# taiyaki-go/motioncheck_ccm_slam

Measured on AMD Instinct MI355X. Metric: ORB extract+match Mfeatures/s and GBA iter/s (2k KF, 200k pts) @1/2/4/8 GPU, higher is better.
Workload: dtype u8; 1 GPU; configs[1]: 256 synthetic 752x480 frames per GPU, 8-level pyramid, 1000 features, FAST+quadtree+rBRIEF, then 1000x1000 brute-force Hamming on the 255 consecutive pairs; frames_per_gpu=256

## Files before the change

motioncheck_ccm_slam_amd/csrc/orb_fast_cells.hip:

```cpp
#include <hip/hip_runtime.h>
#include "orb_types.h"
#include "orb_device.h"

#ifndef FC_NZ
#define FC_NZ 1024
#endif
#ifndef FC_KEPT
#define FC_KEPT 480
#endif
#define FC_CELLS 32
#ifndef FC_TPB
#define FC_TPB 256
#endif
static_assert(FC_TPB == FC_ITEM_STRIDE, "the band record carries the item steps of FC_WAVES waves (fc_enum, orb_device.h)");
#define FC_WAVE_CAP 320
__host__ __device__ inline size_t fc_lds_bytes(int pitch, int bh)
{
    return 2 * (size_t)pitch * bh + (size_t)FC_WAVE_CAP * (FC_TPB / 64) * 2 + 32 + FC_NZ * 2 + FC_KEPT * 4 + FC_CELLS * 16 + 64 * 8 + 256 + 64;
}

__device__ __forceinline__ unsigned fc_u(fc_us2 x) { return __builtin_bit_cast(unsigned, x); }
__device__ __forceinline__ int fc_mbcnt(unsigned long long m, int base)
{
    return (int)__builtin_amdgcn_mbcnt_hi((unsigned)(m >> 32), __builtin_amdgcn_mbcnt_lo((unsigned)m, (unsigned)base));
}
#ifdef FC_STAMPS
#define FC_STAMP_SLOTS 16
#define FC_STAMP_WGS (1 << 17)
__device__ unsigned long long fc_stamps[FC_STAMP_WGS * FC_STAMP_SLOTS];
#define FC_STAMP(k) do { if (threadIdx.x == 0 || threadIdx.x == FC_TPB - 1) { const unsigned wg__ = blockIdx.y * gridDim.x + blockIdx.x; if (wg__ < FC_STAMP_WGS) fc_stamps[wg__ * FC_STAMP_SLOTS + (threadIdx.x ? 8 : 0) + (k)] = __builtin_amdgcn_s_memtime(); } } while (0)
extern "C" int ccm_debug_fc_stamps(unsigned long long* out, int n_wgs)
{
    return hipMemcpyFromSymbol(out, HIP_SYMBOL(fc_stamps), (size_t)n_wgs * FC_STAMP_SLOTS * 8, 0, hipMemcpyDeviceToHost) == hipSuccess ? 0 : -1;
}
#else
#define FC_STAMP(k) do { } while (0)
#endif
typedef const __attribute__((address_space(1))) uint8_t fc_gbyte;
typedef const __attribute__((address_space(1))) unsigned fc_gu32;
typedef const __attribute__((address_space(3))) uint8_t fc_lbyte;
typedef unsigned fc_u32x4 __attribute__((ext_vector_type(4)));
typedef fc_u32x4 fc_u32x4_a4 __attribute__((aligned(4)));
struct FcLate {
    int ini_th, min_th, ncells, slots_per_frame;
    const OrbCell* cells; unsigned* slots; int* cell_count;
    int* clear_status;
};
__global__ __launch_bounds__(FC_TPB) __attribute__((amdgpu_waves_per_eu(8, 8))) void k_fast_cells(const OrbBand* __restrict__ bands, int xcd_on, unsigned grid_x, unsigned grid_y, int frame0,
                                                    const uint8_t* __restrict__ img0, long long plane0, int pitch0, const FcLate g)
{
    extern __shared__ __attribute__((aligned(16))) uint8_t fc_smem[];
    int wx, wy;
    xcd_work_item(xcd_on, grid_x, grid_y, wx, wy);
    FC_STAMP(0);
    const OrbBand B = bands[wx];
#ifdef FC_STAMPS
    asm volatile("s_waitcnt lgkmcnt(0)" ::: "memory");
#endif
    FC_STAMP(6);
    int bclo[4], bcwd[4], bsfirst[4], bscap[4];
#pragma unroll
    for (int i = 0; i < 4; i++) {
        bclo[i] = B.clo[i]; bcwd[i] = B.cwd[i]; bsfirst[i] = B.slot_first[i]; bscap[i] = B.slot_cap[i];
        asm volatile("" : "+s"(bclo[i]), "+s"(bcwd[i]), "+s"(bsfirst[i]), "+s"(bscap[i]));
    }
    int bxa = B.xa, by0 = B.y0, bncells = B.ncells, bcfirst = B.cell_first;
    asm volatile("" : "+s"(bxa), "+s"(by0), "+s"(bncells), "+s"(bcfirst));
    unsigned pw_inv = B.pw_inv, pq_inv = B.pq_inv;
    asm volatile("" : "+s"(pw_inv), "+s"(pq_inv));
    const int f = wy + frame0, tid = threadIdx.x, lane = lane_id(), wv = tid >> 6;
    const bool lvl0 = B.level == 0;
    const uint8_t* const Limg = lvl0 ? img0 : B.img;
    const long long Lplane = lvl0 ? plane0 : B.plane;
    const int Lpitch = lvl0 ? pitch0 : B.lpitch, Lw = B.w, Lh = B.h;
    const int P = B.pitch, bh = B.bh, PW = P >> 2;
    uint8_t* T = fc_smem;
    uint8_t* S = fc_smem + (size_t)P * bh;
    constexpr int NW = FC_TPB / 64;
    const int WCAP = FC_WAVE_CAP;
    unsigned short* surv = reinterpret_cast<unsigned short*>(S + (size_t)P * bh);
    int* nsurv = reinterpret_cast<int*>(surv + NW * WCAP);
    unsigned short* nz = reinterpret_cast<unsigned short*>(nsurv + 8);
    unsigned* kept = reinterpret_cast<unsigned*>(nz + FC_NZ);
    int* cell_hi = reinterpret_cast<int*>(kept + FC_KEPT);
    int* cell_n = cell_hi + FC_CELLS;
    int* cell_k = cell_n + FC_CELLS;
    uint2* colmask = reinterpret_cast<uint2*>(cell_k + FC_CELLS + FC_CELLS);
    uint8_t* colcell = reinterpret_cast<uint8_t*>(colmask + 64);
    int* l_clo = reinterpret_cast<int*>(colcell + 256); int* l_cwd = l_clo + 4; int* l_sfirst = l_cwd + 4; int* l_scap = l_sfirst + 4;
    const uint8_t* img = Limg + (long long)f * Lplane;
    const bool dword_ok = ((reinterpret_cast<uintptr_t>(img) | (uintptr_t)Lpitch) & 3) == 0 && Lpitch >= ((Lw + 3) & ~3);
#ifdef FC_STAMPS
    asm volatile("s_waitcnt lgkmcnt(0)" ::: "memory");
#endif
    FC_STAMP(5);
    fc_gbyte* const gimg = (fc_gbyte*)img;
    const OrbBand* const brec = bands + wx;
    auto under_trip = [&]() {
        if (g.clear_status && (blockIdx.x | blockIdx.y | threadIdx.x) == 0) *g.clear_status = 0;
        const int k = FC_TPB - 1 - tid;
        if (k < FC_CELLS) {
            cell_hi[k] = 0; cell_n[k] = 0; cell_k[k] = 0;
            if (k < 2) nsurv[1 + k] = 0;
            if (k < ORB_BAND_CELLS) { l_clo[k] = brec->clo[k]; l_cwd[k] = brec->cwd[k]; l_sfirst[k] = brec->slot_first[k]; l_scap[k] = brec->slot_cap[k]; }
        }
    };
    if (dword_ok && (P & 15) == 0) {
        const int wmax = ((Lw - 1) & ~3);
        const int PQ = P >> 4, nq = bh * PQ;
        auto chunk = [&](int i) {
            const int ly = (int)(((unsigned)i * pq_inv) >> 20), lq = i - ly * PQ;
            const int gy = min(B.y0 + ly, Lh - 1), gx = B.xa + 16 * lq;
            fc_gbyte* rowp = gimg + (long long)gy * Lpitch;
            fc_u32x4 v;
            if (gx + 12 <= wmax) v = *reinterpret_cast<const __attribute__((address_space(1))) fc_u32x4_a4*>(rowp + gx);
            else {
                v.x = *reinterpret_cast<fc_gu32*>(rowp + min(gx, wmax));
                v.y = *reinterpret_cast<fc_gu32*>(rowp + min(gx + 4, wmax));
                v.z = *reinterpret_cast<fc_gu32*>(rowp + min(gx + 8, wmax));
                v.w = *reinterpret_cast<fc_gu32*>(rowp + min(gx + 12, wmax));
            }
            return v;
        };
        fc_u32x4 v0 = { 0u, 0u, 0u, 0u };
        if (tid < nq) v0 = chunk(tid);
        asm volatile("" ::: "memory");
        under_trip();
        if (tid < nq) {
            reinterpret_cast<fc_u32x4*>(T)[tid] = v0;
            reinterpret_cast<uint4*>(S)[tid] = make_uint4(0u, 0u, 0u, 0u);
        }
        for (int i = tid + FC_TPB; i < nq; i += FC_TPB) {
            const fc_u32x4 v = chunk(i);
            reinterpret_cast<fc_u32x4*>(T)[i] = v;
            reinterpret_cast<uint4*>(S)[i] = make_uint4(0u, 0u, 0u, 0u);
        }
    } else if (dword_ok) {
        const int wmax = ((Lw - 1) & ~3);
        for (int i = tid; i < bh * PW; i += FC_TPB) {
            const int ly = (int)(((unsigned)i * pw_inv) >> 20), lx = i - ly * PW;
            const int gy = min(B.y0 + ly, Lh - 1), gx = min(B.xa + 4 * lx, wmax);
            reinterpret_cast<unsigned*>(T)[i] = *reinterpret_cast<fc_gu32*>(gimg + (long long)gy * Lpitch + gx);
            reinterpret_cast<unsigned*>(S)[i] = 0u;
        }
        under_trip();
    } else {
        for (int i = tid; i < bh * P; i += FC_TPB) {
            const int ly = i / P, lx = i - ly * P;
            const int gy = min(B.y0 + ly, Lh - 1), gx = min(B.xa + lx, Lw - 1);
            T[i] = gimg[(long long)gy * Lpitch + gx];
            S[i] = 0;
        }
        under_trip();
    }
#ifdef FC_STAMPS
    asm volatile("s_waitcnt vmcnt(0)" ::: "memory");
#endif
    FC_STAMP(7);
    const int c_lo = B.c_lo, c_hi = B.c_hi;
    const int t_lo = min(g.ini_th, g.min_th);
    const int dw_lo = B.dw_lo;
    if (tid < PW) {
        unsigned mk[4];
        for (int i = 0; i < 4; i++) mk[i] = (4 * tid + i >= c_lo && 4 * tid + i < c_hi) ? 0xFFFFu : 0u;
        colmask[tid] = make_uint2(mk[0] | (mk[2] << 16), mk[1] | (mk[3] << 16));
    }
    __syncthreads();
    FC_STAMP(1);
    if (tid < P) {
        int ci = 255;
#pragma unroll
        for (int i = 0; i < ORB_BAND_CELLS; i++) if (i < bncells && tid >= bclo[i] && tid < bclo[i] + bcwd[i]) ci = i;
        colcell[tid] = (uint8_t)ci;
    }
    const int wvs = __builtin_amdgcn_readfirstlane(wv);
    unsigned short* wsurv = surv + wvs * WCAP;
    const unsigned t_lds = (unsigned)(uintptr_t)(fc_lbyte*)T;
    const int thr = max(t_lo, 1);
    int wcnt = 0;
    auto score_top = [&]() {
        wcnt = __builtin_amdgcn_readfirstlane(wcnt);
        const int n = min(wcnt, 64);
        wcnt -= n;
        const bool on = lane < n;
        const unsigned long long on_mask = n >= 64 ? ~0ull : (1ull << n) - 1ull;
        const unsigned popped = wsurv[wcnt + lane];
        const unsigned ent = on ? popped : (unsigned)(3 * P + 3);
        const int pos = (int)(ent & 0x7FFFu);
        int rb[7];
#pragma unroll
        for (int k = 0; k < 7; k++) rb[k] = pos + (int)(t_lds + (unsigned)((k - 3) * P - 3));
#define FC_PX(dx, dy) (*(fc_lbyte*)(uintptr_t)(unsigned)(rb[(dy) + 3] + ((dx) + 3)))
        const int v = FC_PX(0, 0);
        int r[16];
        r[0] = FC_PX(0, 3);    r[1] = FC_PX(1, 3);    r[2] = FC_PX(2, 2);    r[3] = FC_PX(3, 1);
        r[4] = FC_PX(3, 0);    r[5] = FC_PX(3, -1);   r[6] = FC_PX(2, -2);   r[7] = FC_PX(1, -3);
        r[8] = FC_PX(0, -3);   r[9] = FC_PX(-1, -3);  r[10] = FC_PX(-2, -2); r[11] = FC_PX(-3, -1);
        r[12] = FC_PX(-3, 0);  r[13] = FC_PX(-3, 1);  r[14] = FC_PX(-2, 2);  r[15] = FC_PX(-1, 3);
#undef FC_PX
        auto store = [&](bool st, int arc) {
            if (st) {
                S[pos] = (uint8_t)(arc - 1);
                const int q = atomicAdd(nsurv + 1, 1);
                if (q < FC_NZ) nz[q] = (unsigned short)pos;
            }
        };
        if (t_lo < 0) {
            const int arc = fast_score16(v, r) + 1;
            store(on && arc > thr, arc);
            return;
        }
        bool again;
        const int arc = fast_arc16_split(v, r, t_lo, (ent >> 15) != 0u, &again);
        store(on && arc > thr, arc);
        const unsigned long long mb = __ballot(again) & on_mask;
        if (mb != 0ull) {
            if (on && again) wsurv[fc_mbcnt(mb, wcnt)] = (unsigned short)(ent | 0x8000u);
            wcnt += __popcll(mb);
            __builtin_amdgcn_fence(__ATOMIC_RELEASE, "wavefront");
        }
    };
    {
        const int n_dw = B.items.n_dw, d_step = B.items.d_step, r_step = B.items.r_step;
        const int runs = fc_item_runs(bh, n_dw), dw_end = dw_lo + n_dw;
        FcItem item = fc_item_start(dw_lo, n_dw, B.items.nd_inv, wv, lane);
        for (int run = wvs; run < runs; run += FC_WAVES) {
            wcnt = __builtin_amdgcn_readfirstlane(wcnt);
            const int pos0 = fc_item_pos0(item, P);
            unsigned kk0 = 0, kk1 = 0;
            if (fc_item_valid(item, bh)) {
                const unsigned* crow = reinterpret_cast<const unsigned*>(T + pos0);
                const unsigned c0 = crow[-1], c1 = crow[0], c2 = crow[1];
                const unsigned nn = crow[3 * PW], ss = crow[-3 * PW];
                const fc_us2 tt = fc_pk((unsigned)t_lo * 0x00010001u);
                unsigned kk[2];
#pragma unroll
                for (int h = 0; h < 2; h++) {
                    const unsigned sel = h ? 0x0c030c01u : 0x0c020c00u;
                    const fc_us2 v = fc_pk(__builtin_amdgcn_perm(0u, c1, sel));
                    const fc_us2 n = fc_pk(__builtin_amdgcn_perm(0u, nn, sel)), sq = fc_pk(__builtin_amdgcn_perm(0u, ss, sel));
                    const fc_us2 w = fc_pk(__builtin_amdgcn_perm(c1, c0, h ? 0x0c040c02u : 0x0c030c01u));
                    const fc_us2 e = fc_pk(__builtin_amdgcn_perm(c2, c1, h ? 0x0c060c04u : 0x0c050c03u));
                    const fc_us2 bm = __builtin_elementwise_min(__builtin_elementwise_max(n, sq), __builtin_elementwise_max(e, w));
                    const fc_us2 dm = __builtin_elementwise_max(__builtin_elementwise_min(n, sq), __builtin_elementwise_min(e, w));
                    kk[h] = fc_u(__builtin_elementwise_sub_sat(bm, (fc_us2)(v + tt))) | fc_u(__builtin_elementwise_sub_sat(__builtin_elementwise_sub_sat(v, tt), dm));
                }
                const uint2 cm = colmask[item.dw];
                kk0 = kk[0] & cm.x; kk1 = kk[1] & cm.y;
            }
            fc_item_step(item, dw_end, n_dw, d_step, r_step);
            const bool k0 = (kk0 & 0xFFFFu) != 0u, k1 = (kk1 & 0xFFFFu) != 0u;
            const bool k2 = (kk0 >> 16) != 0u, k3 = (kk1 >> 16) != 0u;
            const unsigned long long m0 = __ballot(k0), m1 = __ballot(k1), m2 = __ballot(k2), m3 = __ballot(k3);
            if ((m0 | m1 | m2 | m3) != 0ull) {
                const int b1 = wcnt + __popcll(m0), b2 = b1 + __popcll(m1), b3 = b2 + __popcll(m2);
                if (k0) (wsurv + wcnt)[fc_mbcnt(m0, 0)] = (unsigned short)pos0;
                if (k1) (wsurv + b1)[fc_mbcnt(m1, 0)] = (unsigned short)(pos0 + 1);
                if (k2) (wsurv + b2)[fc_mbcnt(m2, 0)] = (unsigned short)(pos0 + 2);
                if (k3) (wsurv + b3)[fc_mbcnt(m3, 0)] = (unsigned short)(pos0 + 3);
                wcnt = b3 + __popcll(m3);
                __builtin_amdgcn_fence(__ATOMIC_RELEASE, "wavefront");
            }
            const int leave = run + FC_WAVES < runs ? 63 : 0;
            while (wcnt > leave) score_top();
        }
    }
    __syncthreads();
    FC_STAMP(2);
    const int nnz = nsurv[1];
    const int rh = bh - 6;
    bool listed = g.min_th <= g.ini_th && nnz <= FC_NZ && bncells <= ORB_BAND_CELLS;
    if (listed) {
        const int cap_c = ((FC_KEPT / max(bncells, 1)) - 1) | 1;
        const unsigned p_inv = 0xFFFFFFFFu / (unsigned)P + 1u;
        for (int e = tid; e < nnz; e += FC_TPB) {
            const int pos = nz[e];
            const int row = (int)__umulhi((unsigned)pos, p_inv), col = pos - row * P;
            const uint8_t* p = S + pos;
            const int ci = colcell[col];
            const int sc = p[0];
            const int nl = p[-1], nr = p[1], nul = p[-P - 1], nu = p[-P], nur = p[-P + 1], ndl = p[P - 1], nd = p[P], ndr = p[P + 1];
            __builtin_amdgcn_sched_barrier(0);
            if (ci == 255) continue;
            const int xx = col - l_clo[ci], yy = row - 3, rw = l_cwd[ci];
            const bool l = xx > 0, r = xx + 1 < rw, u = yy > 0, d = yy + 1 < rh;
#define NB(c, v) ((c) ? (v) : 0)
            const bool keep = (sc > NB(l, nl)) & (sc > NB(r, nr)) &
                              (sc > NB(u && l, nul)) & (sc > NB(u, nu)) & (sc > NB(u && r, nur)) &
                              (sc > NB(d && l, ndl)) & (sc > NB(d, nd)) & (sc > NB(d && r, ndr));
#undef NB
            if (keep) {
                const int q = atomicAdd(cell_k + ci, 1);
                if (q < cap_c) kept[ci * cap_c + q] = ((unsigned)yy << 14) | ((unsigned)xx << 8) | (unsigned)sc;
                if (sc >= g.ini_th) atomicAdd(cell_hi + ci, 1);
            }
        }
        __syncthreads();
        FC_STAMP(3);
        const int4 ck = *reinterpret_cast<const int4*>(cell_k);
        const int e1 = ck.x, e2 = e1 + ck.y, e3 = e2 + ck.z, nk = e3 + ck.w;
        listed = max(max(ck.x, ck.y), max(ck.z, ck.w)) <= cap_c;
        if (listed) {
            if (tid >= FC_TPB - FC_CELLS && FC_TPB - 1 - tid < bncells) {
                const int ci = FC_TPB - 1 - tid;
                const int hi = cell_hi[ci];
                g.cell_count[(long long)f * g.ncells + bcfirst + ci] = hi > 0 ? hi : cell_k[ci];
            }
            for (int e = tid; e < nk; e += FC_TPB) {
                const int ci = (e >= e1 ? 1 : 0) + (e >= e2 ? 1 : 0) + (e >= e3 ? 1 : 0);
                const int k0 = e - (ci == 0 ? 0 : ci == 1 ? e1 : ci == 2 ? e2 : e3);
                const unsigned* bucket = kept + ci * cap_c;
                const int nb = ci == 0 ? ck.x : ci == 1 ? ck.y : ci == 2 ? ck.z : ck.w;
                const unsigned me = bucket[k0];
                const unsigned th = (unsigned)(cell_hi[ci] > 0 ? g.ini_th : g.min_th);
                if ((me & 255u) < th) continue;
                int rank = 0;
                for (int k = 0; k < nb; k++) {
                    const unsigned o = bucket[k];
                    rank += ((o & 255u) >= th && (o >> 8) < (me >> 8)) ? 1 : 0;
                }
                if (rank < l_scap[ci])
                    g.slots[(long long)f * g.slots_per_frame + l_sfirst[ci] + rank] =
                        ((me & 255u) << 24) | ((unsigned)(by0 + 3 - ORB_BORDER + (int)((me >> 14) & 63u)) << 12) |
                        (unsigned)(bxa + l_clo[ci] - ORB_BORDER + (int)((me >> 8) & 63u));
            }
            FC_STAMP(4);
            return;
        }
    }
    for (int ci = wv; ci < B.ncells; ci += FC_TPB / 64) {
        const OrbCell c = g.cells[B.cell_first + ci];
        const int rw = c.cw - 6, rh = c.ch - 6;
        int* count_out = g.cell_count + (long long)f * g.ncells + B.cell_first + ci;
        if (rw <= 0 || rh <= 0) { if (lane == 0) *count_out = 0; continue; }
        const uint8_t* S0 = S + 3 * P + (c.x0 + 3 - B.xa);
        unsigned* out = g.slots + (long long)f * g.slots_per_frame + c.slot_first;
        const int relx = c.x0 + 3 - ORB_BORDER, rely = c.y0 + 3 - ORB_BORDER;
        const int rpi = rw <= 32 ? 2 : 1;
        const int xx = rpi == 2 ? (lane & 31) : lane, yoff = rpi == 2 ? (lane >> 5) : 0;
        int n = 0;
        for (int attempt = 0; attempt < 2 && n == 0; attempt++) {
            const int th = attempt == 0 ? g.ini_th : g.min_th;
            for (int y0 = 0; y0 < rh; y0 += rpi) {
                const int yy = y0 + yoff;
                const bool in = yy < rh && xx < rw;
                const uint8_t* p = S0 + min(yy, rh - 1) * P + min(xx, rw - 1);
                const int s = in ? p[0] : 0;
                if (__ballot(s >= th && s > 0) == 0ull) continue;
                bool keep = false;
                if (s >= th && s > 0) {
                    const bool l = xx > 0, r = xx + 1 < rw, u = yy > 0, d = yy + 1 < rh;
#define NB(c, o) ((c) && (int)p[o] >= th ? (int)p[o] : 0)
                    keep = s > NB(l, -1) && s > NB(r, 1) &&
                           s > NB(u && l, -P - 1) && s > NB(u, -P) && s > NB(u && r, -P + 1) &&
                           s > NB(d && l, P - 1) && s > NB(d, P) && s > NB(d && r, P + 1);
#undef NB
                }
                const unsigned long long m = __ballot(keep);
                if (keep) {
                    const int pos = n + __popcll(m & lanemask_lt());
                    if (pos < c.slot_cap)
                        out[pos] = ((unsigned)s << 24) | ((unsigned)(rely + yy) << 12) | (unsigned)(relx + xx);
                }
                n += __popcll(m);
            }
        }
        if (lane == 0) *count_out = n;
    }
}

void orb_launch_fast_cells(hipStream_t s, const OrbGeom& g_dev, const OrbCell* cells, const OrbBand* bands, int nbands, int nframes,
                           size_t lds_bytes, unsigned* slots, int* cell_count, int* clear_status)
{
    static const int xcd_on = getenv("CCM_ORB_XCD") ? atoi(getenv("CCM_ORB_XCD")) : 0;
    const FcLate late = { g_dev.ini_th, g_dev.min_th, g_dev.ncells, g_dev.slots_per_frame, cells, slots, cell_count, clear_status };
    hipLaunchKernelGGL(k_fast_cells, dim3(nbands, nframes), dim3(FC_TPB), lds_bytes, s, bands, xcd_on, (unsigned)nbands, (unsigned)nframes, g_dev.frame0,
                       g_dev.lv[0].img, g_dev.lv[0].plane, g_dev.lv[0].pitch, late);
}
size_t orb_fast_cells_lds(int pitch, int bh) { return fc_lds_bytes(pitch, bh); }
```

motioncheck_ccm_slam_amd/csrc/orb_host.cpp:

```cpp
#include "ccm_internal.h"
#include "orb_types.h"
#include "orb_device.h"
#include <cmath>
#include <cfloat>
#include <algorithm>

namespace {

inline int cv_round(float v) { return (int)lrintf(v); }
inline int cv_round(double v) { return (int)lrint(v); }

struct OrbTables {
    float scale[ORB_MAX_LEVELS], inv_scale[ORB_MAX_LEVELS], sigma2[ORB_MAX_LEVELS], inv_sigma2[ORB_MAX_LEVELS];
    int nfeat[ORB_MAX_LEVELS];
    int umax[16];
};

int make_tables(const ccm_orb_params* p, OrbTables* t)
{
    if (!p || p->nlevels < 1 || p->nlevels > ORB_MAX_LEVELS || p->nfeatures < 0 || !(p->scale_factor > 1.0f)) return CCM_E_ARG;
    const int n = p->nlevels;
    t->scale[0] = 1.0f; t->sigma2[0] = 1.0f;
    for (int i = 1; i < n; i++) {
        t->scale[i] = t->scale[i - 1] * p->scale_factor;
// ... 129 lines not shown
        L.splane = (long long)L.spitch * L.h;
        S.smap_off[l] = smap_bytes; smap_bytes += align_up((size_t)L.splane * nframes, 256);
        if (l > 0) {
            L.pitch = (int)align_up(L.w, 64);
            L.plane = (long long)L.pitch * L.h;
            S.pyr_off[l] = pyr_bytes; pyr_bytes += align_up((size_t)L.plane * nframes, 256);
            std::vector<int> xo, yo; std::vector<short> xa, ya;
            linear_tables(G.lv[l - 1].w, L.w, xo, xa);
            linear_tables(G.lv[l - 1].h, L.h, yo, ya);
            toff[l].xofs = tab_i.size(); tab_i.insert(tab_i.end(), xo.begin(), xo.end());
            toff[l].yofs = tab_i.size(); tab_i.insert(tab_i.end(), yo.begin(), yo.end());
            toff[l].xab = tab_s.size(); tab_s.insert(tab_s.end(), xa.begin(), xa.end());
            toff[l].yab = tab_s.size(); tab_s.insert(tab_s.end(), ya.begin(), ya.end());
        }
        const int minBX = ORB_BORDER, minBY = ORB_BORDER, maxBX = L.w - ORB_EDGE + 3, maxBY = L.h - ORB_EDGE + 3;
        const float width = (float)(maxBX - minBX), height = (float)(maxBY - minBY);
        const int nCols = (int)(width / 30.f), nRows = (int)(height / 30.f);
        L.bw = maxBX - minBX; L.bh = maxBY - minBY;
        L.cell_first = (int)S.cells.size();
        int key_cap = 0;
        if (nCols >= 1 && nRows >= 1) {
            const int wCell = (int)std::ceil(width / nCols), hCell = (int)std::ceil(height / nRows);
            for (int i = 0; i < nRows; i++) {
                const float iniY = (float)(minBY + i * hCell);
                float maxY = iniY + hCell + 6;
                if (iniY >= maxBY - 3) continue;
                if (maxY > maxBY) maxY = (float)maxBY;
                for (int j = 0; j < nCols; j++) {
                    const float iniX = (float)(minBX + j * wCell);
                    float maxX = iniX + wCell + 6;
                    if (iniX >= maxBX - 6) continue;
                    if (maxX > maxBX) maxX = (float)maxBX;
                    OrbCell cell{};
                    cell.level = (short)l; cell.x0 = (short)iniX; cell.y0 = (short)iniY;
                    cell.cw = (short)((int)maxX - (int)iniX); cell.ch = (short)((int)maxY - (int)iniY);
                    if (cell.cw > 65 || cell.ch > 65)
                        return ccm_fail(c, CCM_E_ARG, "FAST cell %dx%d exceeds the kernel tile", cell.cw, cell.ch);
                    const int rw = std::max(cell.cw - 6, 0), rh = std::max(cell.ch - 6, 0);
                    cell.slot_cap = ((rw + 1) / 2) * ((rh + 1) / 2);
                    cell.slot_first = slot_acc;
                    slot_acc += cell.slot_cap; key_cap += cell.slot_cap;
                    S.cells.push_back(cell);
                }
            }
        }
        L.ncells = (int)S.cells.size() - L.cell_first;
        L.roots = (int)std::round((float)(maxBX - minBX) / (maxBY - minBY));
        if (L.roots < 1 || L.roots > ORB_MAX_ROOTS)
            return ccm_fail(c, CCM_E_ARG, "level %d aspect ratio gives %d quadtree roots (1..%d supported)", l, L.roots, ORB_MAX_ROOTS);
        L.hx = (float)(maxBX - minBX) / L.roots;
        L.key_first = key_acc; L.key_cap = std::max(key_cap, 1); key_acc += L.key_cap;
        L.out_cap = std::max(L.quota + 4, 4 * L.roots);
        L.out_first = out_acc; out_acc += L.out_cap;
        L.tiles_x = (L.w + 63) / 64; L.tiles_y = (L.h + 63) / 64;
        L.tile_first = tile_acc; tile_acc += L.tiles_x * L.tiles_y;
    }
    S.bands.clear(); S.band_lds = 0;
    static const bool want_fused = !(getenv("CCM_ORB_FUSED") && atoi(getenv("CCM_ORB_FUSED")) == 0);
    S.fused = want_fused;
    constexpr int pcap = 144;
    for (size_t a = 0; a < S.cells.size();) {
        size_t b = a;
        const OrbCell& c0 = S.cells[a];
        const int xa = (c0.x0 - 4) & ~3;
        int pitch = 0;
        while (b < S.cells.size() && S.cells[b].level == c0.level && S.cells[b].y0 == c0.y0) {
            const int p2 = (int)align_up((size_t)(S.cells[b].x0 + S.cells[b].cw + 4 - xa), 16);
            if (b > a && (p2 > pcap || b - a >= ORB_BAND_CELLS)) break;
            pitch = p2; b++;
        }
        OrbBand band{};
        band.cell_first = (int)a; band.ncells = (int)(b - a); band.level = c0.level; band.xa = (short)xa; band.y0 = (short)c0.y0;
        band.pitch = (short)pitch; band.bh = (short)c0.ch;
        {
            const OrbCell& cl = S.cells[b - 1];
            const int PW = pitch / 4, PQ = std::max(pitch / 16, 1);
            band.c_lo = (short)(c0.x0 + 3 - xa); band.c_hi = (short)(cl.x0 + cl.cw - 3 - xa);
            band.dw_lo = (short)std::max(1, band.c_lo >> 2); band.dw_hi = (short)std::min(PW - 2, (band.c_hi - 1) >> 2);
            band.pw_inv = (1u << 20) / (unsigned)PW + 1u; band.pq_inv = (1u << 20) / (unsigned)PQ + 1u;
            band.items = fc_enum(band.dw_lo, band.dw_hi);
            band.w = G.lv[c0.level].w; band.h = G.lv[c0.level].h;
            for (size_t k = a; k < b; k++) {
                const OrbCell& ck = S.cells[k];
                band.clo[k - a] = (short)(ck.x0 + 3 - xa); band.cwd[k - a] = (short)(ck.cw - 6);
                band.slot_first[k - a] = ck.slot_first; band.slot_cap[k - a] = ck.slot_cap;
            }
        }
        for (size_t k = a; k < b; k++) if (S.cells[k].ch != c0.ch) S.fused = false;
        S.bands.push_back(band);
        a = b;
    }
    for (const OrbBand& b : S.bands) S.band_lds = std::max(S.band_lds, orb_fast_cells_lds(b.pitch, b.bh));
    for (const OrbBand& b : S.bands) if (b.pitch > 256) S.fused = false;
    if (S.band_lds > 60 * 1024) S.fused = false;
    for (const OrbBand& b : S.bands) if ((int)b.pitch * b.bh >= (1 << 15)) S.fused = false;
    G.ncells = (int)S.cells.size(); G.ntiles = tile_acc;
    G.slots_per_frame = std::max(slot_acc, 1); G.keys_per_frame = key_acc; G.out_per_frame = out_acc;
    int list_cap = 0;
    for (int l = 0; l < p->nlevels; l++) list_cap = std::max(list_cap, G.lv[l].out_cap);
    G.list_cap = (int)align_up(list_cap + 4, 16);
    if (orb_octree_lds_bytes(G.list_cap) > 150 * 1024)
        return ccm_fail(c, CCM_E_ARG, "nfeatures too large for the quadtree kernel's LDS (list cap %d)", G.list_cap);
    if (max_per_image < 1) return ccm_fail(c, CCM_E_ARG, "max_per_image must be positive");

    CCM_RESERVE(c, S.pyr, std::max<size_t>(pyr_bytes, 256));
    CCM_RESERVE(c, S.smap, smap_bytes);
    CCM_RESERVE(c, S.slots, (size_t)G.slots_per_frame * nframes * 4);
    CCM_RESERVE(c, S.cell_count, (size_t)std::max(G.ncells, 1) * nframes * 4);
    CCM_RESERVE(c, S.keysA, (size_t)G.keys_per_frame * nframes * 4);
    CCM_RESERVE(c, S.keysB, (size_t)G.keys_per_frame * nframes * 4);
    CCM_RESERVE(c, S.sel, (size_t)G.out_per_frame * nframes * 4);
    CCM_RESERVE(c, S.sel_count, (size_t)p->nlevels * nframes * 4);
    CCM_RESERVE(c, S.status, 256);
    CCM_RESERVE(c, S.kps, (size_t)nframes * max_per_image * sizeof(ccm_keypoint));
    CCM_RESERVE(c, S.desc, (size_t)nframes * max_per_image * 32);
    CCM_RESERVE(c, S.counts, (size_t)nframes * 4);
    const size_t tab_bytes = align_up(tab_i.size() * 4, 16) + tab_s.size() * 2;
    CCM_RESERVE(c, S.tables_dev, std::max<size_t>(tab_bytes, 16));
    CCM_RESERVE(c, S.cells_dev, std::max<size_t>(S.cells.size(), 1) * sizeof(OrbCell));
    CCM_RESERVE(c, S.bands_dev, std::max<size_t>(S.bands.size(), 1) * sizeof(OrbBand));
    CCM_RESERVE(c, S.geom_dev, sizeof(OrbGeom));
    char* tb = S.tables_dev.as<char>();
    const size_t s_base = align_up(tab_i.size() * 4, 16);
    for (int l = 0; l < p->nlevels; l++) {
        OrbLevel& L = G.lv[l];
        L.smap = S.smap.as<uint8_t>() + S.smap_off[l];
        if (l > 0) {
            L.img = S.pyr.as<uint8_t>() + S.pyr_off[l];
            L.xofs = reinterpret_cast<const int*>(tb) + toff[l].xofs;
            L.yofs = reinterpret_cast<const int*>(tb) + toff[l].yofs;
            L.xab = reinterpret_cast<const short*>(tb + s_base) + toff[l].xab;
            L.yab = reinterpret_cast<const short*>(tb + s_base) + toff[l].yab;
        }
    }
    if (!tab_i.empty()) CCM_HIP(c, hipMemcpyAsync(tb, tab_i.data(), tab_i.size() * 4, hipMemcpyHostToDevice, c->stream));
    if (!tab_s.empty()) CCM_HIP(c, hipMemcpyAsync(tb + s_base, tab_s.data(), tab_s.size() * 2, hipMemcpyHostToDevice, c->stream));
    if (!S.cells.empty())
        CCM_HIP(c, hipMemcpyAsync(S.cells_dev.p, S.cells.data(), S.cells.size() * sizeof(OrbCell), hipMemcpyHostToDevice, c->stream));
    for (OrbBand& b : S.bands) {
        const OrbLevel& L = G.lv[b.level];
        b.img = b.level > 0 ? L.img : nullptr; b.plane = L.plane; b.lpitch = L.pitch;
    }
    if (!S.bands.empty())
        CCM_HIP(c, hipMemcpyAsync(S.bands_dev.p, S.bands.data(), S.bands.size() * sizeof(OrbBand), hipMemcpyHostToDevice, c->stream));
    CCM_HIP(c, hipStreamSynchronize(c->stream));
    if (!S.pattern_up) { CCM_HIP(c, orb_upload_pattern()); S.pattern_up = true; }
    S.par = *p; S.w = w; S.h = h; S.nframes = nframes; S.max_per_image = max_per_image;
    S.valid = true;
    S.last_img = nullptr;
    return CCM_OK;
}

static int orb_run(ccm_ctx* c, const uint8_t* img_dev, int stride, size_t image_stride, int frame0 = 0, int nrun = -1,
                   hipStream_t st = nullptr, hipEvent_t first_done = nullptr)
{
    OrbState& S = *c->orb;
    OrbGeom& G = S.geom;
    G.lv[0].img = img_dev; G.lv[0].pitch = stride; G.lv[0].plane = (long long)image_stride;
    G.frame0 = frame0;
    if (nrun < 0) nrun = S.nframes - frame0;
    if (!st) st = c->stream;
    const OrbGeom& gd = G;
    const OrbCell* cd = S.cells_dev.as<OrbCell>();
    int* clear = frame0 == 0 ? S.status.as<int>() : nullptr;
    for (int l = 1; l < G.nlevels; l++) {
        ProfScope ps(c, CCM_PROF_RESIZE);
        orb_launch_resize(st, gd, l, G.lv[l].w, G.lv[l].h, nrun, clear);
        clear = nullptr;
        if (l == 1 && first_done) CCM_HIP(c, hipEventRecord(first_done, st));
    }
    if (S.fused && !S.bands.empty()) {
        ProfScope ps(c, CCM_PROF_FAST_SCORE);
        orb_launch_fast_cells(st, gd, cd, S.bands_dev.as<OrbBand>(), (int)S.bands.size(), nrun, S.band_lds, S.slots.as<unsigned>(), S.cell_count.as<int>(), clear);
        if (G.nlevels == 1 && first_done) CCM_HIP(c, hipEventRecord(first_done, st));
    } else {
        if (clear) CCM_HIP(c, hipMemsetAsync(clear, 0, 4, st));
        { ProfScope ps(c, CCM_PROF_FAST_SCORE); orb_launch_score(st, gd, G.ntiles, nrun); }
        if (G.ncells > 0) { ProfScope ps(c, CCM_PROF_CELL_NMS); orb_launch_nms(st, gd, cd, G.ncells, nrun, S.slots.as<unsigned>(), S.cell_count.as<int>()); }
    }
    { ProfScope ps(c, CCM_PROF_OCTREE);
    orb_launch_octree(st, gd, cd, G.nlevels, nrun, G.list_cap, S.slots.as<unsigned>(), S.cell_count.as<int>(),
                      S.keysA.as<unsigned>(), S.keysB.as<unsigned>(), S.sel.as<unsigned>(), S.sel_count.as<int>(),
                      S.status.as<int>()); }
    { ProfScope ps(c, CCM_PROF_ORIENT_DESC);
    orb_launch_orient_desc(st, gd, G.out_per_frame, nrun, S.sel.as<unsigned>(), S.sel_count.as<int>(),
                           S.kps.as<ccm_keypoint>(), S.desc.as<uint8_t>(), S.counts.as<int>(), S.max_per_image,
                           S.status.as<int>()); }
    CCM_HIP(c, hipGetLastError());
    S.have_result = true;
    return CCM_OK;
}

static int orb_extract_lanes(ccm_ctx* c, const uint8_t* img_dev, int stride, size_t image_stride)
{
    OrbState& S = *c->orb;
    static const int lane_env = getenv("CCM_ORB_LANE_FRAMES") ? std::max(0, atoi(getenv("CCM_ORB_LANE_FRAMES"))) : -1;
    const int lane_frames = lane_env >= 0 ? lane_env : std::max(128, orb_switch_frames(S.geom.out_per_frame));
    const bool one_lane = c->prof_on || !S.fused || S.bands.empty();
    const std::vector<OrbChunk> plan = orb_lane_plan(S.nframes, S.geom.out_per_frame, one_lane ? 0 : lane_frames);
    if (plan.size() < 2) return orb_run(c, img_dev, stride, image_stride);
    if (!S.lane_join) {
        if (!(S.lane_stream = ccm_aux_stream(c, 1))) return ccm_fail(c, CCM_E_DEVICE, "hipStreamCreate failed");
        for (hipEvent_t* e : { &S.lane_fork, &S.lane_join })
            if (!*e) CCM_HIP(c, hipEventCreateWithFlags(e, hipEventDisableTiming));
    }
    int rc = CCM_OK;
    bool forked = false;
    for (size_t k = 0; k < plan.size() && rc == CCM_OK; k++) {
        const OrbChunk& ck = plan[k];
        if (k == 1) {
            hipError_t e = hipStreamWaitEvent(S.lane_stream, S.lane_fork, 0);
            if (e != hipSuccess) { rc = ccm_fail(c, CCM_E_DEVICE, "hipStreamWaitEvent -> %s", hipGetErrorString(e)); break; }
            forked = true;
        }
        rc = orb_run(c, img_dev, stride, image_stride, ck.frame0, ck.nrun, ck.lane ? S.lane_stream : c->stream, k == 0 ? S.lane_fork : nullptr);
    }
    if (forked) {
        hipError_t e = hipEventRecord(S.lane_join, S.lane_stream);
        if (e == hipSuccess) e = hipStreamWaitEvent(c->stream, S.lane_join, 0);
        if (e != hipSuccess) {
            (void)hipStreamSynchronize(S.lane_stream);
            if (rc == CCM_OK) rc = ccm_fail(c, CCM_E_DEVICE, "joining the extractor's lanes -> %s", hipGetErrorString(e));
        }
    }
    return rc;
}

static int orb_check_status(ccm_ctx* c)
{
    OrbState& S = *c->orb;
    int st = 0;
    CCM_HIP(c, hipMemcpyAsync(&st, S.status.p, 4, hipMemcpyDeviceToHost, c->stream));
    CCM_HIP(c, hipStreamSynchronize(c->stream));
    if (st & 8) return ccm_fail(c, CCM_E_CAPACITY, "an image produced more than max_per_image keypoints");
    if (st) return ccm_fail(c, CCM_E_DEVICE, "extractor kernel status 0x%x (1 key overflow, 2 quadtree guard, 4 list overflow)", st);
    return CCM_OK;
}

int orb_last_result(ccm_ctx* c, const ccm_keypoint** kps, const uint8_t** desc, const int32_t** counts, int* n_images, int* max_per_image,
                    int* nlevels)
{
    if (!c->orb || !c->orb->have_result) return ccm_fail(c, CCM_E_STATE, "no extraction on this context yet");
    const OrbState& S = *c->orb;
    *kps = S.kps.as<ccm_keypoint>(); *desc = S.desc.as<uint8_t>(); *counts = S.counts.as<int32_t>();
    *n_images = S.nframes; *max_per_image = S.max_per_image; *nlevels = S.par.nlevels;
    return CCM_OK;
}

extern "C" {

int ccm_orb_tables(const ccm_orb_params* p, float* scale, float* inv_scale, float* sigma2, float* inv_sigma2,
                   int32_t* features_per_level, int32_t* umax)
{
    OrbTables t;
    int rc = make_tables(p, &t);
    if (rc) return rc;
    for (int i = 0; i < p->nlevels; i++) {
        if (scale) scale[i] = t.scale[i];
        if (inv_scale) inv_scale[i] = t.inv_scale[i];
        if (sigma2) sigma2[i] = t.sigma2[i];
        if (inv_sigma2) inv_sigma2[i] = t.inv_sigma2[i];
        if (features_per_level) features_per_level[i] = t.nfeat[i];
    }
    if (umax) for (int i = 0; i < 16; i++) umax[i] = t.umax[i];
    return CCM_OK;
}

int ccm_orb_level_sizes(const ccm_orb_params* p, int w, int h, int32_t* level_w, int32_t* level_h)
{
    OrbTables t;
    int rc = make_tables(p, &t);
    if (rc) return rc;
    if (!level_w || !level_h) return CCM_E_ARG;
    for (int l = 0; l < p->nlevels; l++) {
        level_w[l] = cv_round((float)w * t.inv_scale[l]);
        level_h[l] = cv_round((float)h * t.inv_scale[l]);
    }
    return CCM_OK;
}

int ccm_orb_extract_dev(ccm_ctx* c, const ccm_orb_params* p, const uint8_t* img_dev, int w, int h, int stride,
                        size_t image_stride, int n_images, int max_per_image)
{
    RoctxRange roctx_("ccm_orb_extract_dev");
    return ccm_guard(c, "ccm_orb_extract_dev", [&]() -> int {
        if (!c || !p) return CCM_E_ARG;
        if (n_images == 0 || w == 0 || h == 0) return CCM_OK;
        if (!img_dev || w < 0 || h < 0 || n_images < 0 || stride < w || (n_images > 1 && image_stride < (size_t)stride * h))
            return ccm_fail(c, CCM_E_ARG, "bad image arguments");
        CCM_HIP(c, hipSetDevice(c->device));
        int rc = orb_prepare(c, p, w, h, n_images, max_per_image);
        if (rc) return rc;
        return orb_extract_lanes(c, img_dev, stride, image_stride);
    });
}

int ccm_orb_debug_lane_plan(int n_images, int out_per_frame, int lane_frames, int32_t* frame0, int32_t* nrun, int32_t* lane, int max)
{
    return ccm_guard(nullptr, "ccm_orb_debug_lane_plan", [&]() -> int {
        if (n_images < 0 || out_per_frame < 1 || lane_frames < 0 || max < 0) return CCM_E_ARG;
        const std::vector<OrbChunk> plan = orb_lane_plan(n_images, out_per_frame, lane_frames);
        for (size_t k = 0; k < plan.size() && k < (size_t)max; k++) {
            if (frame0) frame0[k] = plan[k].frame0;
            if (nrun) nrun[k] = plan[k].nrun;
            if (lane) lane[k] = plan[k].lane;
        }
        return (int)plan.size();
    });
}

int ccm_orb_fetch(ccm_ctx* c, ccm_keypoint* kps, uint8_t* desc, int32_t* counts)
{
    RoctxRange roctx_("ccm_orb_fetch");
    if (!c || !c->orb || !c->orb->have_result) return c ? ccm_fail(c, CCM_E_STATE, "no extraction to fetch") : CCM_E_ARG;
    OrbState& S = *c->orb;
    int rc = orb_check_status(c);
    if (rc) return rc;
    if (kps) CCM_HIP(c, hipMemcpyAsync(kps, S.kps.p, (size_t)S.nframes * S.max_per_image * sizeof(ccm_keypoint), hipMemcpyDeviceToHost, c->stream));
    if (desc) CCM_HIP(c, hipMemcpyAsync(desc, S.desc.p, (size_t)S.nframes * S.max_per_image * 32, hipMemcpyDeviceToHost, c->stream));
    if (counts) CCM_HIP(c, hipMemcpyAsync(counts, S.counts.p, (size_t)S.nframes * 4, hipMemcpyDeviceToHost, c->stream));
    CCM_HIP(c, hipStreamSynchronize(c->stream));
    return CCM_OK;
}

int ccm_orb_extract(ccm_ctx* c, const ccm_orb_params* p, const uint8_t* img, int w, int h, int stride,
                    size_t image_stride, int n_images, ccm_keypoint* kps, uint8_t* desc, int32_t* counts,
                    int max_per_image)
{
    RoctxRange roctx_("ccm_orb_extract");
    return ccm_guard(c, "ccm_orb_extract", [&]() -> int {
        if (!c || !p) return CCM_E_ARG;
        if (n_images == 0 || w == 0 || h == 0) return CCM_OK;
        if (!img || w < 0 || h < 0 || n_images < 0 || stride < w) return ccm_fail(c, CCM_E_ARG, "bad image arguments");
        CCM_HIP(c, hipSetDevice(c->device));
        if (!c->orb) c->orb = new OrbState();
        OrbState& S = *c->orb;
        static const bool force_2d = getenv("CCM_ORB_UPLOAD_2D") && atoi(getenv("CCM_ORB_UPLOAD_2D")) != 0;
        static const int chunk_frames = getenv("CCM_ORB_CHUNK") ? std::max(1, atoi(getenv("CCM_ORB_CHUNK"))) : 64;
        const int n_chunks = n_images >= 2 * chunk_frames ? (n_images + chunk_frames - 1) / chunk_frames : 1;
        const bool linear = !force_2d && n_chunks > 1 && stride % 16 == 0 && image_stride % 16 == 0 && image_stride >= (size_t)stride * h;
        const int pitch = linear ? stride : (int)align_up(w, 64);
        const size_t plane = linear ? image_stride : (size_t)pitch * h;
        CCM_RESERVE(c, S.img0, plane * n_images + 64);
        int rc = orb_prepare(c, p, w, h, n_images, max_per_image);
        if (rc) return rc;
        if (n_chunks > 1 && !S.copy_stream) {
            if (!(S.copy_stream = ccm_aux_stream(c, 0))) return ccm_fail(c, CCM_E_DEVICE, "hipStreamCreate failed");
            CCM_HIP(c, hipEventCreateWithFlags(&S.copy_done, hipEventDisableTiming));
        }
        const bool contiguous = n_images == 1 || image_stride == (size_t)stride * h;
        auto page_locked = [](const void* q) {
            if (!q) return true;
            hipPointerAttribute_t a{};
            if (hipPointerGetAttributes(&a, q) != hipSuccess) { (void)hipGetLastError(); return false; }
            return a.type == hipMemoryTypeHost;
        };
        const bool stream_down = n_chunks > 1 && (kps || desc || counts) && page_locked(kps) && page_locked(desc) && page_locked(counts);
        if (stream_down && !S.down_stream) {
            if (!(S.down_stream = ccm_aux_stream(c, 1))) return ccm_fail(c, CCM_E_DEVICE, "hipStreamCreate failed");
            CCM_HIP(c, hipEventCreateWithFlags(&S.chunk_done, hipEventDisableTiming));
        }
        for (int ck = 0; ck < n_chunks; ck++) {
            const int f0 = (int)((long long)n_images * ck / n_chunks), f1 = (int)((long long)n_images * (ck + 1) / n_chunks);
            hipStream_t up = n_chunks > 1 ? S.copy_stream : c->stream;
            if (linear) {
                const size_t bytes = f1 < n_images ? plane * (f1 - f0) : plane * (f1 - 1 - f0) + (size_t)stride * (h - 1) + w;
                CCM_HIP(c, hipMemcpyAsync(S.img0.as<char>() + plane * f0, img + image_stride * f0, bytes, hipMemcpyHostToDevice, up));
            } else if (contiguous) {
// ... 126 lines not shown
```

Measured before the change: 332.9 Mfeatures/s.

## Precompute column cell flags, prefetch first nz entry, and rebalance extractor lanes

In the fused FAST kernel, the per-column cell byte now also stores left and right border flags. The kept-record format stores the absolute column, so the per-candidate lookups of cell origin and width in LDS are dropped, and slot first/cap are packed into one int2. The first nz entry is loaded before the listed loop, row division uses a reciprocal already in scope, and cap_c is selected from constants instead of a runtime divide. On the host, lane chunks alternate between streams so the last chunk lands on the main stream, and the first chunk can hand its post-resize work to another stream. This trades more complex stream logic for less per-candidate ALU and LDS work.

```diff
diff --git a/motioncheck_ccm_slam_amd/csrc/orb_fast_cells.hip b/motioncheck_ccm_slam_amd/csrc/orb_fast_cells.hip
--- a/motioncheck_ccm_slam_amd/csrc/orb_fast_cells.hip
+++ b/motioncheck_ccm_slam_amd/csrc/orb_fast_cells.hip
@@ -87,7 +87,8 @@
     int* cell_k = cell_n + FC_CELLS;
     uint2* colmask = reinterpret_cast<uint2*>(cell_k + FC_CELLS + FC_CELLS);
     uint8_t* colcell = reinterpret_cast<uint8_t*>(colmask + 64);
-    int* l_clo = reinterpret_cast<int*>(colcell + 256); int* l_cwd = l_clo + 4; int* l_sfirst = l_cwd + 4; int* l_scap = l_sfirst + 4;
+    int2* l_slot = reinterpret_cast<int2*>(colcell + 256);
+    const OrbBand* const brec = bands + wx;
     const uint8_t* img = Limg + (long long)f * Lplane;
     const bool dword_ok = ((reinterpret_cast<uintptr_t>(img) | (uintptr_t)Lpitch) & 3) == 0 && Lpitch >= ((Lw + 3) & ~3);
 #ifdef FC_STAMPS
@@ -95,14 +96,13 @@
 #endif
     FC_STAMP(5);
     fc_gbyte* const gimg = (fc_gbyte*)img;
-    const OrbBand* const brec = bands + wx;
     auto under_trip = [&]() {
         if (g.clear_status && (blockIdx.x | blockIdx.y | threadIdx.x) == 0) *g.clear_status = 0;
         const int k = FC_TPB - 1 - tid;
         if (k < FC_CELLS) {
             cell_hi[k] = 0; cell_n[k] = 0; cell_k[k] = 0;
             if (k < 2) nsurv[1 + k] = 0;
-            if (k < ORB_BAND_CELLS) { l_clo[k] = brec->clo[k]; l_cwd[k] = brec->cwd[k]; l_sfirst[k] = brec->slot_first[k]; l_scap[k] = brec->slot_cap[k]; }
+            if (k < ORB_BAND_CELLS) l_slot[k] = make_int2(brec->slot_first[k], brec->slot_cap[k]);
         }
     };
     if (dword_ok && (P & 15) == 0) {
@@ -168,10 +168,13 @@
     __syncthreads();
     FC_STAMP(1);
     if (tid < P) {
-        int ci = 255;
+        int ci = 255, lo = 0, hi = 0;
 #pragma unroll
-        for (int i = 0; i < ORB_BAND_CELLS; i++) if (i < bncells && tid >= bclo[i] && tid < bclo[i] + bcwd[i]) ci = i;
-        colcell[tid] = (uint8_t)ci;
+        for (int i = 0; i < ORB_BAND_CELLS; i++) {
+            const bool in = i < bncells && tid >= bclo[i] && tid < bclo[i] + bcwd[i];
+            ci = in ? i : ci; lo = in ? bclo[i] : lo; hi = in ? bclo[i] + bcwd[i] : hi;
+        }
+        colcell[tid] = (uint8_t)(ci | (tid > lo && tid < hi ? 4 : 0) | (tid + 1 < hi ? 8 : 0));
     }
     const int wvs = __builtin_amdgcn_readfirstlane(wv);
     unsigned short* wsurv = surv + wvs * WCAP;
@@ -267,23 +270,28 @@
     }
     __syncthreads();
     FC_STAMP(2);
+    static_assert(FC_TPB <= FC_NZ, "nz[tid] is read before nnz is known");
     const int nnz = nsurv[1];
+    int nz0 = nz[tid];
+    asm volatile("" : "+v"(nz0));
     const int rh = bh - 6;
     bool listed = g.min_th <= g.ini_th && nnz <= FC_NZ && bncells <= ORB_BAND_CELLS;
     if (listed) {
-        const int cap_c = ((FC_KEPT / max(bncells, 1)) - 1) | 1;
-        const unsigned p_inv = 0xFFFFFFFFu / (unsigned)P + 1u;
+        static_assert(ORB_BAND_CELLS == 4, "cap_c by cell count");
+#define FC_CAP(n) (((FC_KEPT / (n)) - 1) | 1)
+        const int cap_c = bncells <= 1 ? FC_CAP(1) : bncells == 2 ? FC_CAP(2) : bncells == 3 ? FC_CAP(3) : FC_CAP(4);
+#undef FC_CAP
         for (int e = tid; e < nnz; e += FC_TPB) {
-            const int pos = nz[e];
-            const int row = (int)__umulhi((unsigned)pos, p_inv), col = pos - row * P;
+            const int pos = e == tid ? nz0 : nz[e];
+            const int row = (int)(((unsigned)(pos >> 2) * pw_inv) >> 20), col = pos - row * P;
             const uint8_t* p = S + pos;
-            const int ci = colcell[col];
+            const int cc = colcell[col];
             const int sc = p[0];
             const int nl = p[-1], nr = p[1], nul = p[-P - 1], nu = p[-P], nur = p[-P + 1], ndl = p[P - 1], nd = p[P], ndr = p[P + 1];
             __builtin_amdgcn_sched_barrier(0);
-            if (ci == 255) continue;
-            const int xx = col - l_clo[ci], yy = row - 3, rw = l_cwd[ci];
-            const bool l = xx > 0, r = xx + 1 < rw, u = yy > 0, d = yy + 1 < rh;
+            if (cc == 255) continue;
+            const int ci = cc & 3, yy = row - 3;
+            const bool l = (cc & 4) != 0, r = (cc & 8) != 0, u = yy > 0, d = yy + 1 < rh;
 #define NB(c, v) ((c) ? (v) : 0)
             const bool keep = (sc > NB(l, nl)) & (sc > NB(r, nr)) &
                               (sc > NB(u && l, nul)) & (sc > NB(u, nu)) & (sc > NB(u && r, nur)) &
@@ -291,7 +299,7 @@
 #undef NB
             if (keep) {
                 const int q = atomicAdd(cell_k + ci, 1);
-                if (q < cap_c) kept[ci * cap_c + q] = ((unsigned)yy << 14) | ((unsigned)xx << 8) | (unsigned)sc;
+                if (q < cap_c) kept[ci * cap_c + q] = ((unsigned)yy << 16) | ((unsigned)col << 8) | (unsigned)sc;
                 if (sc >= g.ini_th) atomicAdd(cell_hi + ci, 1);
             }
         }
@@ -319,10 +327,11 @@
                     const unsigned o = bucket[k];
                     rank += ((o & 255u) >= th && (o >> 8) < (me >> 8)) ? 1 : 0;
                 }
-                if (rank < l_scap[ci])
-                    g.slots[(long long)f * g.slots_per_frame + l_sfirst[ci] + rank] =
-                        ((me & 255u) << 24) | ((unsigned)(by0 + 3 - ORB_BORDER + (int)((me >> 14) & 63u)) << 12) |
-                        (unsigned)(bxa + l_clo[ci] - ORB_BORDER + (int)((me >> 8) & 63u));
+                const int2 sl = l_slot[ci];
+                if (rank < sl.y)
+                    g.slots[(long long)f * g.slots_per_frame + sl.x + rank] =
+                        ((me & 255u) << 24) | ((unsigned)(by0 + 3 - ORB_BORDER + (int)((me >> 16) & 63u)) << 12) |
+                        (unsigned)(bxa - ORB_BORDER + (int)((me >> 8) & 255u));
             }
             FC_STAMP(4);
             return;
diff --git a/motioncheck_ccm_slam_amd/csrc/orb_host.cpp b/motioncheck_ccm_slam_amd/csrc/orb_host.cpp
--- a/motioncheck_ccm_slam_amd/csrc/orb_host.cpp
+++ b/motioncheck_ccm_slam_amd/csrc/orb_host.cpp
@@ -305,7 +305,7 @@
 }
 
 static int orb_run(ccm_ctx* c, const uint8_t* img_dev, int stride, size_t image_stride, int frame0 = 0, int nrun = -1,
-                   hipStream_t st = nullptr, hipEvent_t first_done = nullptr)
+                   hipStream_t st = nullptr, hipEvent_t first_done = nullptr, hipStream_t rest = nullptr)
 {
     OrbState& S = *c->orb;
     OrbGeom& G = S.geom;
@@ -313,6 +313,7 @@
     G.frame0 = frame0;
     if (nrun < 0) nrun = S.nframes - frame0;
     if (!st) st = c->stream;
+    if (!rest || !first_done) rest = st;
     const OrbGeom& gd = G;
     const OrbCell* cd = S.cells_dev.as<OrbCell>();
     int* clear = frame0 == 0 ? S.status.as<int>() : nullptr;
@@ -320,12 +321,18 @@
         ProfScope ps(c, CCM_PROF_RESIZE);
         orb_launch_resize(st, gd, l, G.lv[l].w, G.lv[l].h, nrun, clear);
         clear = nullptr;
-        if (l == 1 && first_done) CCM_HIP(c, hipEventRecord(first_done, st));
+        if (l == 1 && first_done) {
+            CCM_HIP(c, hipEventRecord(first_done, st));
+            if (rest != st) { CCM_HIP(c, hipStreamWaitEvent(rest, first_done, 0)); st = rest; }
+        }
     }
     if (S.fused && !S.bands.empty()) {
         ProfScope ps(c, CCM_PROF_FAST_SCORE);
         orb_launch_fast_cells(st, gd, cd, S.bands_dev.as<OrbBand>(), (int)S.bands.size(), nrun, S.band_lds, S.slots.as<unsigned>(), S.cell_count.as<int>(), clear);
-        if (G.nlevels == 1 && first_done) CCM_HIP(c, hipEventRecord(first_done, st));
+        if (G.nlevels == 1 && first_done) {
+            CCM_HIP(c, hipEventRecord(first_done, st));
+            if (rest != st) { CCM_HIP(c, hipStreamWaitEvent(rest, first_done, 0)); st = rest; }
+        }
     } else {
         if (clear) CCM_HIP(c, hipMemsetAsync(clear, 0, 4, st));
         { ProfScope ps(c, CCM_PROF_FAST_SCORE); orb_launch_score(st, gd, G.ntiles, nrun); }
@@ -361,12 +368,18 @@
     bool forked = false;
     for (size_t k = 0; k < plan.size() && rc == CCM_OK; k++) {
         const OrbChunk& ck = plan[k];
-        if (k == 1) {
+        hipStream_t st = ((plan.size() - 1 - k) & 1) ? S.lane_stream : c->stream;
+        if (k == 0) {
+            forked = st != c->stream;
+            rc = orb_run(c, img_dev, stride, image_stride, ck.frame0, ck.nrun, c->stream, S.lane_fork, st);
+            continue;
+        }
+        if (st != c->stream && !forked) {
             hipError_t e = hipStreamWaitEvent(S.lane_stream, S.lane_fork, 0);
             if (e != hipSuccess) { rc = ccm_fail(c, CCM_E_DEVICE, "hipStreamWaitEvent -> %s", hipGetErrorString(e)); break; }
             forked = true;
         }
-        rc = orb_run(c, img_dev, stride, image_stride, ck.frame0, ck.nrun, ck.lane ? S.lane_stream : c->stream, k == 0 ? S.lane_fork : nullptr);
+        rc = orb_run(c, img_dev, stride, image_stride, ck.frame0, ck.nrun, st);
     }
     if (forked) {
         hipError_t e = hipEventRecord(S.lane_join, S.lane_stream);
```

New measurement: 337.3 Mfeatures/s (median of 6 runs). +1.3%, better.
